# AllenNeuralDynamics/aind-exaspim-image-compression

Hardware: AMD Instinct MI355X
Metric: denoised+encoded voxels/s on 1024^3 uint16 (higher is better)
Workload: dtype f32

## Files before the change

aind-exaspim-image-compression_amd/csrc/bm_kernels.hip:

```cpp
#include "exabm4d_kernels.h"
#include <type_traits>

namespace exabm4d {

struct __attribute__((packed, aligned(4))) float4u {
    float x, y, z, w;
};

constexpr int TCZ = 8;
constexpr int NE = 6;
constexpr int NSTEP = SWIN * 2 * 4;
template <int TCY_, int TCX_>
struct TilePlan {
    static constexpr int TCY = TCY_, TCX = TCX_;
    static constexpr int TRY = TCY - 1, TRX = TCX - 1;
    static constexpr int PROWS = 4 * (TCY - 1) + 3 + NE;
    static_assert(TCY * TCX == 64, "one wave per cell layer");
};
template <int TCY_, int TCX_>
struct TileShape : TilePlan<TCY_, TCX_> {
    using Plan = TilePlan<TCY_, TCX_>;
    static constexpr int PCOLS = 4 * (TCX_ - 1) + 16;
    static constexpr int PSTR = TCX_ == 8 ? 56 : PCOLS;
    static constexpr int PCH = PSTR / 4;
    static constexpr int NDMA = (Plan::PROWS * PCH + 63) / 64;
    static constexpr int PLANE = (Plan::PROWS * PSTR + 3) / 4 * 4;
    static constexpr int PBUF = PLANE > 2144 ? PLANE : 2144;
    static_assert(PCOLS % 4 == 0 && PSTR % 4 == 0, "whole 16-byte chunks");
};

constexpr int CARRY_ROUND = (NE / 2) * SWIN * 64;
constexpr int CARRY_TILE = (NSTEP / 4) * 2 * CARRY_ROUND;
struct Carry {
    int on;
    int strip;
    uint32_t* buf;
    int* done;
    int* ticket;
    unsigned* status;
    int fault;
};
constexpr int CARRY_POLL_LIMIT = 1 << 23;
template <class T>
__device__ __forceinline__ void carry_prefetch(const T* src, T* dst, int lane) {
    static_assert(2 * CARRY_ROUND == 16 * 256 + 128, "two rounds = 16.5 KB");
#pragma unroll
    for (int i = 0; i < 16; i++)
        __builtin_amdgcn_global_load_lds((const __attribute__((address_space(1))) void*)(src + 256 * i + 4 * lane),
                                         (__attribute__((address_space(3))) void*)(dst + 256 * i), 16, 0, 17);
    if (lane < 32)
        __builtin_amdgcn_global_load_lds((const __attribute__((address_space(1))) void*)(src + 4096 + 4 * lane),
                                         (__attribute__((address_space(3))) void*)(dst + 4096), 16, 0, 17);
}
__device__ __forceinline__ void carry_wait_for(const int* done, int tiles, int lane, const Carry& carry) {
    if (lane == 0) {
        int polls = carry.fault ? CARRY_POLL_LIMIT : 0;
        while (__hip_atomic_load(done, __ATOMIC_RELAXED, __HIP_MEMORY_SCOPE_SYSTEM) < tiles) {
            if (++polls > CARRY_POLL_LIMIT) {
                __hip_atomic_fetch_or(carry.status, 1u, __ATOMIC_RELAXED, __HIP_MEMORY_SCOPE_SYSTEM);
                break;
            }
            __builtin_amdgcn_s_sleep(32);
        }
        if (carry.fault) __hip_atomic_fetch_or(carry.status, 1u, __ATOMIC_RELAXED, __HIP_MEMORY_SCOPE_SYSTEM);
    }
}
__device__ __forceinline__ int launch_position(const Carry& carry, int quota) {
    if (!carry.on) return (int)blockIdx.x;
    __shared__ int s_pos;
    if (threadIdx.x == 0) {
        const int xcc = (int)(__builtin_amdgcn_s_getreg((4 - 1) << 11 | 0 << 6 | 20) & 7);
        int pos = -1;
        for (int k = 0; k < 8 && pos < 0; k++) {
            const int c = (xcc + k) & 7;
            const int j = __hip_atomic_fetch_add(carry.ticket + c, 1, __ATOMIC_RELAXED, __HIP_MEMORY_SCOPE_AGENT);
            if (j < quota) pos = 8 * j + c;
        }
        s_pos = pos;
    }
    __syncthreads();
    return s_pos;
}

struct TileId {
    int tz, col, cols;
    int bi, ty, tx;
};
__device__ __forceinline__ bool tile_id(TileId& t, int tiles_y, int tiles_x, int xcd_q, int nbatch,
                                        const Carry& carry) {
    const int per = tiles_y * tiles_x;
    t.cols = per * nbatch;
    if (xcd_q) {
        const int lp = launch_position(carry, (int)(gridDim.x >> 3));
        const int s = lp < 0 ? -1 : xcd_slab_sync(lp, t.cols, xcd_q);
        if (s < 0) return false;
        t.tz = s / t.cols;
        t.col = s - t.tz * t.cols;
    } else {
        const int s = xcd_contiguous(blockIdx.x, gridDim.x);
        t.tz = s / per;
        t.col = (int)blockIdx.y * per + (s - t.tz * per);
    }
    t.bi = t.col / per;
    const int pos = t.col - t.bi * per;
    int ty, tx;
    if (carry.strip) {
        const int sidx = pos / (carry.strip * tiles_x), r = pos - sidx * (carry.strip * tiles_x);
        const int h = min(carry.strip, tiles_y - sidx * carry.strip);
        tx = r / h;
        ty = sidx * carry.strip + (r - tx * h);
    } else {
        ty = pos / tiles_x;
        tx = pos - ty * tiles_x;
    }
    t.ty = ty;
    t.tx = tx;
    return true;
}

__device__ __forceinline__ void list_admit(uint32_t (&list)[MAXG], uint32_t& thr, uint32_t keymax, uint32_t sbits,
                                           uint32_t code, bool valid) {
    uint32_t key = (sbits & KEY_DMASK) | code;
    key = valid ? key : KEY_EMPTY;
    if (__any(key < thr)) {
        const uint32_t kins = key < thr ? key : KEY_EMPTY;
        list_insert_inplace(list, kins);
        thr = min(list[MAXG - 1], keymax);
    }
}
__device__ __forceinline__ void list_store(uint32_t* out, uint32_t (&list)[MAXG]) {
    list[0] = list[0] == KEY_EMPTY ? 0u : list[0];
#pragma unroll
    for (int k = 0; k < MAXG; k += 4) {
        uint4 v = make_uint4(list[k], list[k + 1], list[k + 2], list[k + 3]);
        *reinterpret_cast<uint4*>(out + k) = v;
    }
}

template <class TS>
__global__ __launch_bounds__(512) void bm_tile_kernel(const float* __restrict__ vol_all, VolGeom g,
                                                      uint32_t keymax,
                                                      uint32_t* __restrict__ keys_all, int tiles_y,
                                                      int tiles_x, int guarded, int xcd_q, int nbatch, Carry carry) {
    constexpr int TCX = TS::TCX, TRX = TS::TRX, TRY = TS::TRY, PROWS = TS::PROWS,
                  PCOLS = TS::PCOLS, PSTR = TS::PSTR, PCH = TS::PCH, NDMA = TS::NDMA, PBUF = TS::PBUF;
    __shared__ __align__(16) float pbuf_all[TCZ][2][PBUF];
    __shared__ __align__(16) float lower0[2 * CARRY_ROUND + 64];

    TileId id;
    if (!tile_id(id, tiles_y, tiles_x, xcd_q, nbatch, carry)) return;
    const int tz = id.tz, col = id.col, cols = id.cols, bi = id.bi, ty = id.ty, tx = id.tx;
    const float* __restrict__ vol = vol_all + (size_t)bi * (size_t)g.nvox;
    uint32_t* __restrict__ keys = keys_all + (size_t)bi * (size_t)g.nref * MAXG;
    const int tid = threadIdx.x;
    const int lane = tid & 63;
    const int cx = lane % TCX, cy = lane / TCX, cz = __builtin_amdgcn_readfirstlane(tid >> 6);
    const int ix = TRX * tx + cx, iy = TRY * ty + cy;

    const size_t sy = (size_t)g.nx, sz = (size_t)g.nx * (size_t)g.ny;

    const int Ls = (carry.on ? TCZ : TCZ - 1) * tz;
    const float* carry_rd = reinterpret_cast<const float*>(carry.buf) + ((size_t)((tz + 1) & 1) * cols + col) * CARRY_TILE;
    float* carry_wr = reinterpret_cast<float*>(carry.buf) + ((size_t)(tz & 1) * cols + col) * CARRY_TILE;
    int* done_col = carry.done + col;

    const int qy = min(STEP * iy, g.ny - STEP), qx = min(STEP * ix, g.nx - STEP);
    const int Y0 = STEP * TRY * ty, X0 = STEP * TRX * tx - RAD;
    const bool xin = guarded || ((X0 >= 0) && (X0 + PCOLS - 1 <= g.nx - 1));

    const bool ref_yx = cx < TRX && cy < TRY && iy < g.ay && ix < g.ax;
    const int ry = STEP * iy, rx = STEP * ix;

    uint32_t xmask = 0;
#pragma unroll
    for (int d = 0; d < SWIN; d++)
        xmask |= ((rx + d - RAD >= 0) && (rx + d - RAD <= g.nx - BLK)) ? (1u << d) : 0u;

    const bool yin = (Y0 - RAD >= 0) && (Y0 + 1 + PROWS - 1 <= g.ny - 1);
    do {
    const int L = Ls + cz;
    const bool active = L <= g.az;
    const int iz = L - 1;
    const int qz = min(STEP * L, g.nz - STEP);
    const int Z0 = STEP * L;
    const bool lower_carried = carry.on && cz == 0 && tz > 0;
    const bool carries = carry.on && cz == TCZ - 1 && L + 1 <= g.az;
    const bool ref_ok = ref_yx && active && (cz > 0 || lower_carried);
    if ((lower_carried || carries) && tz > 0) carry_wait_for(done_col, tz, lane, carry);
    const int rz = STEP * iz;

    uint32_t list[MAXG];
#pragma unroll
    for (int k = 0; k < MAXG; k++) list[k] = KEY_EMPTY;
    uint32_t thr = keymax;

    auto step_plane = [&](int step, int& dylo) -> const float* {
        const int z = step & 3, pass = (step >> 2) & 1, dz = (step >> 3) - RAD;
        dylo = pass == 0 ? -RAD : 1;
        const int pz = min(max(Z0 + z + dz, 0), g.nz - 1);
        return vol + (size_t)pz * sz;
    };
    auto issue_dma = [&](int step, float* dst) {
        int dylo;
        const float* plane = step_plane(step, dylo);
        int l = lane;
        asm volatile("" : "+v"(l));
        if (yin) {
            const float* base = plane + (ptrdiff_t)(Y0 + dylo) * (ptrdiff_t)sy + X0;
#pragma unroll
            for (int i = 0; i < NDMA; i++) {
                const unsigned p = 64u * i + (unsigned)l;
                const unsigned r0 = (p * (65536u / PCH + 1u)) >> 16;
                const unsigned r = min(r0, (unsigned)(PROWS - 1));
                const unsigned q = min(p - r0 * PCH, (unsigned)(PCOLS / 4 - 1));
                const float* src = base + (r * (unsigned)sy + 4u * q);
                if (64 * i + 64 <= PROWS * PCH || p < (unsigned)(PROWS * PCH))
                    __builtin_amdgcn_global_load_lds(
                        (const __attribute__((address_space(1))) void*)src,
                        (__attribute__((address_space(3))) void*)(dst + 256 * i), 16, 0, 0);
            }
            return;
        }
#pragma unroll
        for (int i = 0; i < NDMA; i++) {
            const int p = 64 * i + l;
            const int r = min(p / PCH, PROWS - 1), q = min(p % PCH, PCOLS / 4 - 1);
            const int yy = min(max(Y0 + dylo + r, 0), g.ny - 1);
            const float* src = plane + (size_t)yy * sy + (X0 + 4 * q);
            if (64 * i + 64 <= PROWS * PCH || p < PROWS * PCH)
                __builtin_amdgcn_global_load_lds(
                    (const __attribute__((address_space(1))) void*)src,
                    (__attribute__((address_space(3))) void*)(dst + 256 * i), 16, 0, 0);
        }
    };
    auto stage_edge = [&](int step, float* dst) {
        int dylo;
        const float* plane = step_plane(step, dylo);
        for (int c = lane; c < PROWS * PCOLS; c += 64) {
            const int r = c / PCOLS, q = c - r * PCOLS;
            const int yy = min(max(Y0 + dylo + r, 0), g.ny - 1);
            const int xx = min(max(X0 + q, 0), g.nx - 1);
            dst[r * PSTR + q] = plane[(size_t)yy * sy + xx];
        }
    };

    if (!active) {
        for (int i = 0; i < (NSTEP / 4) * 4; i++) __syncthreads();
        break;
    }

    if (xin)
        issue_dma(0, pbuf_all[cz][0]);
    else
        stage_edge(0, pbuf_all[cz][0]);

    float acc[NE][SWIN];
#pragma unroll
    for (int e = 0; e < NE; e++)
#pragma unroll
        for (int d = 0; d < SWIN; d++) acc[e][d] = 0.0f;

#pragma unroll 1
    for (int step = 0; step < NSTEP; step++) {
        const int z = step & 3, pass = (step >> 2) & 1, dz = (step >> 3) - RAD;
        const int dylo = pass == 0 ? -RAD : 1;
        float* cur = pbuf_all[cz][step & 1];
        float* nxt = pbuf_all[cz][(step + 1) & 1];

        asm volatile("s_waitcnt vmcnt(0)" ::: "memory");
        float A[16];
#pragma unroll
        for (int y = 0; y < 4; y++) {
            const float4u t4 = *reinterpret_cast<const float4u*>(
                vol + (size_t)(qz + z) * sz + (size_t)(qy + y) * sy + qx);
            A[4 * y] = t4.x;
            A[4 * y + 1] = t4.y;
            A[4 * y + 2] = t4.z;
            A[4 * y + 3] = t4.w;
        }
        asm volatile("s_waitcnt vmcnt(0)" ::: "memory");
        if (xin && step + 1 < NSTEP) issue_dma(step + 1, nxt);
        if (lower_carried && z == 2) carry_prefetch(carry_rd + (size_t)(step >> 2) * 2 * CARRY_ROUND, lower0, lane);

        {
            const float* wrow = cur + (4 * cy) * PSTR + 4 * cx;
            float4 wq[4], wn[4];
#pragma unroll
            for (int j = 0; j < 4; j++) wq[j] = *reinterpret_cast<const float4*>(wrow + 4 * j);
#pragma unroll
            for (int rp = 0; rp < 3 + NE; rp++) {
                if (rp + 1 < 3 + NE) {
#pragma unroll
                    for (int j = 0; j < 4; j++)
                        wn[j] = *reinterpret_cast<const float4*>(wrow + (rp + 1) * PSTR + 4 * j);
                }
                asm volatile("" ::: "memory");
                const float w[16] = {wq[0].x, wq[0].y, wq[0].z, wq[0].w, wq[1].x, wq[1].y,
                                     wq[1].z, wq[1].w, wq[2].x, wq[2].y, wq[2].z, wq[2].w,
                                     wq[3].x, wq[3].y, wq[3].z, wq[3].w};
#pragma unroll
                for (int y = 0; y < 4; y++) {
                    const int e = rp - y;
                    if (e >= 0 && e < NE) {
#pragma unroll
                        for (int x = 0; x < 4; x++) {
                            const float a = A[4 * y + x];
#pragma unroll
                            for (int d = 0; d < SWIN; d++) {
                                const float t = a - w[d + x];
                                acc[e][d] = fmaf(t, t, acc[e][d]);
                            }
                        }
                    }
                }
#pragma unroll
                for (int j = 0; j < 4; j++) wq[j] = wn[j];
            }
        }
        asm volatile("" ::: "memory");

        if (z == 3) {
            const bool vz = (rz + dz >= 0) && (rz + dz <= g.nz - BLK);
            float* mine = cur + lane;
            const float* up_w = cur + lane;
            const float* lo_w = (cz > 0 ? pbuf_all[max(cz - 1, 0)][step & 1] : lower0) + lane;
            float* cslot = carry_wr + (size_t)((step >> 2) * 2) * CARRY_ROUND + lane;
#pragma unroll
            for (int e0 = 0; e0 < NE; e0 += NE / 2) {
#pragma unroll
                for (int e = e0; e < e0 + NE / 2; e++)
#pragma unroll
                    for (int d = 0; d < SWIN; d++) {
                        const float right = __int_as_float(__builtin_amdgcn_update_dpp(
                            0, __float_as_int(acc[e][d]), 0x101 , 0xF, 0xF, true));
                        mine[64 * ((e - e0) * SWIN + d)] = acc[e][d] + right;
                    }
                __syncthreads();
                if (ref_ok) {
#pragma unroll
                    for (int e = e0; e < e0 + NE / 2; e++) {
                        const int dy = dylo + e;
                        if (dy <= RAD) {
                            const bool vzy = vz && (ry + dy >= 0) && (ry + dy <= g.ny - BLK);
                            const uint32_t cbase =
                                1u + (uint32_t)(((dz + RAD) * SWIN + (dy + RAD)) * SWIN);
                            const bool self_row = (dz == 0) && (dy == 0);
#pragma unroll
                            for (int d = 0; d < SWIN; d++) {
                                const float* c0 = lo_w + (cz == 0 && e0 ? CARRY_ROUND : 0) + 64 * ((e - e0) * SWIN + d);
                                const float* c1 = up_w + 64 * ((e - e0) * SWIN + d);
                                float s0 = c0[0] + c0[TCX];
                                asm("" : "+v"(s0));
                                const float s1 = c1[0] + c1[TCX];
                                const float S = s0 + s1;
                                const uint32_t code = (d == RAD && self_row) ? 0u : cbase + d;
                                const bool valid = vzy && ((xmask >> d) & 1u);
                                list_admit(list, thr, keymax, __float_as_uint(S), code, valid);
                            }
                        }
                    }
                }
                __syncthreads();
                if (carries) {
#pragma unroll
                    for (int e = e0; e < e0 + NE / 2; e++)
#pragma unroll
                        for (int d = 0; d < SWIN; d++) {
                            const float right = __int_as_float(__builtin_amdgcn_update_dpp(
                                0, __float_as_int(acc[e][d]), 0x101 , 0xF, 0xF, true));
                            __hip_atomic_store(cslot + (e0 ? CARRY_ROUND : 0) + 64 * ((e - e0) * SWIN + d), acc[e][d] + right,
                                               __ATOMIC_RELAXED, __HIP_MEMORY_SCOPE_SYSTEM);
                        }
                }
            }
#pragma unroll
            for (int e = 0; e < NE; e++)
#pragma unroll
                for (int d = 0; d < SWIN; d++) acc[e][d] = 0.0f;
        }

        if (!xin && step + 1 < NSTEP) stage_edge(step + 1, nxt);
    }

    if (ref_ok) list_store(keys + ((size_t)((size_t)iz * g.gy + iy) * g.gx + ix) * MAXG, list);
    } while (false);

    if (carry.on) {
        asm volatile("s_waitcnt vmcnt(0)" ::: "memory");
        __syncthreads();
        if (threadIdx.x == 0) __hip_atomic_store(done_col, tz + 1, __ATOMIC_RELAXED, __HIP_MEMORY_SCOPE_SYSTEM);
    }
}

typedef short s16x2 __attribute__((ext_vector_type(2)));
template <int TCY_, int TCX_>
struct TileShape16 : TilePlan<TCY_, TCX_> {
    using Plan = TilePlan<TCY_, TCX_>;
    static constexpr int PCOLS = ((4 * TCX_ + 10 + 7) / 8) * 8;
    static constexpr int PSTR = TCX_ == 8 ? 56 : 80;
    static constexpr int PCH = PSTR / 8;
    static constexpr int NDMA = (Plan::PROWS * PCH + 63) / 64;
    static constexpr int PLANE_DW = NDMA * 256;
    static constexpr int XCH_DW = (NE / 2) * SWIN * 64;
    static constexpr int PBUF = PLANE_DW > XCH_DW ? PLANE_DW : XCH_DW;
    static_assert(PCOLS <= PSTR, "staged columns fit the row");
};

template <class TS>
__global__ __launch_bounds__(512) void bm_tile16_kernel(const uint16_t* __restrict__ vol_all, VolGeom g,
                                                        uint32_t keymax,
                                                        uint32_t* __restrict__ keys_all, int tiles_y,
                                                        int tiles_x, int xcd_q, int nbatch, Carry carry) {
    constexpr int TCX = TS::TCX, TRX = TS::TRX, TRY = TS::TRY, PROWS = TS::PROWS, PCOLS = TS::PCOLS,
                  PSTR = TS::PSTR, PCH = TS::PCH, NDMA = TS::NDMA, PBUF = TS::PBUF;
    __shared__ __align__(16) uint32_t pbuf_all[TCZ][2][PBUF];
    __shared__ __align__(16) uint32_t lower0[2 * CARRY_ROUND + 64];

    TileId id;
    if (!tile_id(id, tiles_y, tiles_x, xcd_q, nbatch, carry)) return;
    const int tz = id.tz, col = id.col, cols = id.cols, bi = id.bi, ty = id.ty, tx = id.tx;
    const uint16_t* __restrict__ vol = vol_all + (size_t)bi * (size_t)g.nvox;
    uint32_t* __restrict__ keys = keys_all + (size_t)bi * (size_t)g.nref * MAXG;
    const int tid = threadIdx.x;
    const int lane = tid & 63;
    const int cx = lane % TCX, cy = lane / TCX, cz = __builtin_amdgcn_readfirstlane(tid >> 6);
    const int ix = TRX * tx + cx, iy = TRY * ty + cy;
    const size_t sy = (size_t)g.nx, sz = (size_t)g.nx * (size_t)g.ny;

    const int Ls = (carry.on ? TCZ : TCZ - 1) * tz;
    const uint32_t* carry_rd = carry.buf + ((size_t)((tz + 1) & 1) * cols + col) * CARRY_TILE;
    uint32_t* carry_wr = carry.buf + ((size_t)(tz & 1) * cols + col) * CARRY_TILE;
    int* done_col = carry.done + col;

    const int qy = min(STEP * iy, g.ny - STEP), qx = min(STEP * ix, g.nx - STEP);
    const int Y0 = STEP * TRY * ty, X0 = STEP * TRX * tx - RAD - 1;
    const int ry = STEP * iy, rx = STEP * ix;
    const bool ref_yx = cx < TRX && cy < TRY && iy < g.ay && ix < g.ax;

    uint32_t xmask = 0;
#pragma unroll
    for (int d = 0; d < SWIN; d++)
        xmask |= ((rx + d - RAD >= 0) && (rx + d - RAD <= g.nx - BLK)) ? (1u << d) : 0u;
    const bool yin = (Y0 - RAD >= 0) && (Y0 + 1 + PROWS - 1 <= g.ny - 1);

    do {
    const int L = Ls + cz;
    const bool active = L <= g.az;
    const int iz = L - 1;
    const int qz = min(STEP * L, g.nz - STEP);
    const int Z0 = STEP * L;
    const bool lower_carried = carry.on && cz == 0 && tz > 0;
    const bool carries = carry.on && cz == TCZ - 1 && L + 1 <= g.az;
    const bool ref_ok = ref_yx && active && (cz > 0 || lower_carried);
    if ((lower_carried || carries) && tz > 0) carry_wait_for(done_col, tz, lane, carry);
    const int rz = STEP * iz;

    uint32_t list[MAXG];
#pragma unroll
    for (int k = 0; k < MAXG; k++) list[k] = KEY_EMPTY;
    uint32_t thr = keymax;

    auto issue_dma = [&](int step, uint32_t* dst) {
        const int z = step & 3, pass = (step >> 2) & 1, dz = (step >> 3) - RAD;
        const int dylo = pass == 0 ? -RAD : 1;
        const int pz = min(max(Z0 + z + dz, 0), g.nz - 1);
        const uint16_t* plane = vol + (size_t)pz * sz;
        int l = lane;
        asm volatile("" : "+v"(l));
#pragma unroll
        for (int i = 0; i < NDMA; i++) {
            const unsigned p = 64u * i + (unsigned)l;
            const unsigned r0 = (p * (65536u / PCH + 1u)) >> 16;
            const unsigned r = min(r0, (unsigned)(PROWS - 1));
            const unsigned q = min(p - r0 * PCH, (unsigned)(PCOLS / 8 - 1));
            const int yy = yin ? Y0 + dylo + (int)r : min(max(Y0 + dylo + (int)r, 0), g.ny - 1);
            const uint16_t* src = plane + (ptrdiff_t)yy * (ptrdiff_t)sy + (X0 + 8 * (int)q);
            __builtin_amdgcn_global_load_lds(
                (const __attribute__((address_space(1))) void*)src,
                (__attribute__((address_space(3))) void*)(dst + 256 * i), 16, 0, 0);
        }
    };

    if (!active) {
        for (int i = 0; i < (NSTEP / 4) * 4; i++) __syncthreads();
        break;
    }
    issue_dma(0, pbuf_all[cz][0]);

    int acc[NE][SWIN];
#pragma unroll
    for (int e = 0; e < NE; e++)
#pragma unroll
        for (int d = 0; d < SWIN; d++) acc[e][d] = 0;

    auto step_body = [&](auto NEc, const int step) {
        constexpr int NEP = decltype(NEc)::value;
        constexpr int NR0 = (NEP + 1) / 2;
        const int z = step & 3, dz = (step >> 3) - RAD;
        const int dylo = NEP == NE ? -RAD : 1;
        uint32_t* cur = pbuf_all[cz][step & 1];
        uint32_t* nxt = pbuf_all[cz][(step + 1) & 1];

        asm volatile("s_waitcnt vmcnt(0)" ::: "memory");
        uint2 A[4];
#pragma unroll
        for (int y = 0; y < 4; y++) {
            const uint32_t* ap = reinterpret_cast<const uint32_t*>(
                vol + (size_t)(qz + z) * sz + (size_t)(qy + y) * sy + qx);
            A[y] = make_uint2(ap[0], ap[1]);
        }
        asm volatile("s_waitcnt vmcnt(0)" ::: "memory");
        if (step + 1 < NSTEP) issue_dma(step + 1, nxt);
        if (lower_carried && z == 2) carry_prefetch(carry_rd + (size_t)(step >> 2) * 2 * CARRY_ROUND, lower0, lane);

        {
            const uint32_t* wrow = cur + ((4 * cy) * PSTR + 4 * cx) / 2;
            uint2 wq[4], wn[4];
#pragma unroll
            for (int j = 0; j < 4; j++) wq[j] = *reinterpret_cast<const uint2*>(wrow + 2 * j);
#pragma unroll
            for (int rp = 0; rp < 3 + NEP; rp++) {
                if (rp + 1 < 3 + NEP) {
#pragma unroll
                    for (int j = 0; j < 4; j++)
                        wn[j] = *reinterpret_cast<const uint2*>(wrow + (rp + 1) * (PSTR / 2) + 2 * j);
                }
                asm volatile("" ::: "memory");
                const uint32_t W[8] = {wq[0].x, wq[0].y, wq[1].x, wq[1].y, wq[2].x, wq[2].y, wq[3].x, wq[3].y};
                uint32_t Wo[7];
#pragma unroll
                for (int i = 0; i < 7; i++) Wo[i] = __builtin_amdgcn_alignbit(W[i + 1], W[i], 16);
#pragma unroll
                for (int y = 0; y < 4; y++) {
                    const int e = rp - y;
                    if (e >= 0 && e < NEP) {
#pragma unroll
                        for (int xp = 0; xp < 2; xp++) {
                            const s16x2 a = __builtin_bit_cast(s16x2, xp ? A[y].y : A[y].x);
#pragma unroll
                            for (int d = 0; d < SWIN; d++) {
                                const int j = 1 + 2 * xp + d;
                                const uint32_t wp = (j & 1) ? Wo[(j - 1) / 2] : W[j / 2];
                                const s16x2 t = __builtin_elementwise_sub_sat(a, __builtin_bit_cast(s16x2, wp));
                                acc[e][d] = __builtin_amdgcn_sdot2(t, t, acc[e][d], true);
                            }
                        }
                    }
                }
#pragma unroll
                for (int j = 0; j < 4; j++) wq[j] = wn[j];
            }
        }
        asm volatile("" ::: "memory");

        if (z == 3) {
            const bool vz = (rz + dz >= 0) && (rz + dz <= g.nz - BLK);
            uint32_t* mine = cur + lane;
            const uint32_t* up_w = cur + lane;
            const uint32_t* lo_w = (cz > 0 ? pbuf_all[max(cz - 1, 0)][step & 1] : lower0) + lane;
            uint32_t* cslot = carry_wr + (size_t)((step >> 2) * 2) * CARRY_ROUND + lane;
            auto pair_sum = [&](int e, int d) {
                const uint32_t c = min((uint32_t)acc[e][d], 1u << 27);
                const uint32_t right = (uint32_t)__builtin_amdgcn_update_dpp(
                    0, (int)c, 0x101 , 0xF, 0xF, true);
                return c + right;
            };
#pragma unroll
            for (int e0 = 0; e0 < NEP; e0 += NR0) {
#pragma unroll
                for (int e = e0; e < (e0 + NR0 < NEP ? e0 + NR0 : NEP); e++)
#pragma unroll
                    for (int d = 0; d < SWIN; d++) mine[64 * ((e - e0) * SWIN + d)] = pair_sum(e, d);
                __syncthreads();
                if (ref_ok) {
#pragma unroll
                    for (int e = e0; e < (e0 + NR0 < NEP ? e0 + NR0 : NEP); e++) {
                        uint32_t Sv[1][SWIN];
#pragma unroll
                        for (int d = 0; d < SWIN; d++) {
                            const uint32_t* c0 = lo_w + (cz == 0 && e0 ? CARRY_ROUND : 0) + 64 * ((e - e0) * SWIN + d);
                            const uint32_t* c1 = up_w + 64 * ((e - e0) * SWIN + d);
                            Sv[0][d] = (c0[0] + c0[TCX]) + (c1[0] + c1[TCX]);
                        }
                        asm volatile("" ::: "memory");
                        const int dy = dylo + e;
                        {
                            const bool vzy = vz && (ry + dy >= 0) && (ry + dy <= g.ny - BLK);
                            const uint32_t cbase =
                                1u + (uint32_t)(((dz + RAD) * SWIN + (dy + RAD)) * SWIN);
                            const bool self_row = (dz == 0) && (dy == 0);
#pragma unroll
                            for (int d = 0; d < SWIN; d++) {
                                const uint32_t S = Sv[0][d];
                                const uint32_t code = (d == RAD && self_row) ? 0u : cbase + d;
                                const bool valid = vzy && ((xmask >> d) & 1u);
                                list_admit(list, thr, keymax, __float_as_uint((float)S), code, valid);
                            }
                        }
                    }
                }
                __syncthreads();
                if (carries) {
                    uint32_t* cw = cslot + (size_t)(e0 ? CARRY_ROUND : 0);
#pragma unroll
                    for (int e = e0; e < (e0 + NR0 < NEP ? e0 + NR0 : NEP); e++)
#pragma unroll
                        for (int d = 0; d < SWIN; d++)
                            __hip_atomic_store(cw + 64 * ((e - e0) * SWIN + d), pair_sum(e, d), __ATOMIC_RELAXED,
                                               __HIP_MEMORY_SCOPE_SYSTEM);
                }
            }
#pragma unroll
            for (int e = 0; e < NE; e++)
#pragma unroll
                for (int d = 0; d < SWIN; d++) acc[e][d] = 0;
        }
    };
#pragma unroll 1
    for (int step = 0; step < NSTEP; step++) {
        if (((step >> 2) & 1) == 0)
            step_body(std::integral_constant<int, NE>{}, step);
        else
            step_body(std::integral_constant<int, NE - 1>{}, step);
    }

    if (ref_ok) list_store(keys + ((size_t)((size_t)iz * g.gy + iy) * g.gx + ix) * MAXG, list);
    } while (false);

    if (carry.on) {
        asm volatile("s_waitcnt vmcnt(0)" ::: "memory");
        __syncthreads();
        if (threadIdx.x == 0) __hip_atomic_store(done_col, tz + 1, __ATOMIC_RELAXED, __HIP_MEMORY_SCOPE_SYSTEM);
    }
}

__global__ __launch_bounds__(64) void bm_generic_kernel(const float* __restrict__ vol_all,
                                                        VolGeom g, uint32_t keymax,
                                                        uint32_t* __restrict__ keys_all,
                                                        int only_unaligned) {
    __shared__ float rb[BVOX];
    const float* __restrict__ vol = vol_all + (size_t)blockIdx.y * (size_t)g.nvox;
    uint32_t* __restrict__ keys = keys_all + (size_t)blockIdx.y * (size_t)g.nref * MAXG;

    const long long r = blockIdx.x;
    const int ix = (int)(r % g.gx), iy = (int)((r / g.gx) % g.gy),
              iz = (int)(r / ((long long)g.gx * g.gy));
    if (only_unaligned && iz < g.az && iy < g.ay && ix < g.ax) return;
    const int rz = grid_pos(iz, g.az, g.nz), ry = grid_pos(iy, g.ay, g.ny),
              rx = grid_pos(ix, g.ax, g.nx);
    const size_t sy = (size_t)g.nx, sz = (size_t)g.nx * (size_t)g.ny;
    const int lane = threadIdx.x;

    for (int i = lane; i < BVOX; i += 64) {
        const int bx = i & 7, by = (i >> 3) & 7, bz = i >> 6;
        rb[i] = vol[(size_t)(rz + bz) * sz + (size_t)(ry + by) * sy + (rx + bx)];
    }
    __syncthreads();

    uint32_t list[MAXG];
#pragma unroll
    for (int k = 0; k < MAXG; k++) list[k] = KEY_EMPTY;

    for (int c = lane; c < NCAND; c += 64) {
        const int dx = c % SWIN - RAD, dy = (c / SWIN) % SWIN - RAD, dz = c / (SWIN * SWIN) - RAD;
        const int pz = rz + dz, py = ry + dy, px = rx + dx;
        const bool valid = pz >= 0 && pz <= g.nz - BLK && py >= 0 && py <= g.ny - BLK && px >= 0 &&
                           px <= g.nx - BLK;
        uint32_t key = KEY_EMPTY;
        if (valid) {
            const float* __restrict__ b = vol + (size_t)pz * sz + (size_t)py * sy + px;
            float cell[8];
#pragma unroll 1
            for (int kc = 0; kc < 8; kc++) {
                const int kz = kc >> 2, ky = (kc >> 1) & 1, kx = kc & 1;
                float acc = 0.0f;
#pragma unroll 1
                for (int z = 0; z < 4; z++)
#pragma unroll
                    for (int y = 0; y < 4; y++) {
                        const int bz = 4 * kz + z, by = 4 * ky + y;
                        const float* bp = b + (size_t)bz * sz + (size_t)by * sy + 4 * kx;
                        const float* ap = rb + (bz * 8 + by) * 8 + 4 * kx;
#pragma unroll
                        for (int x = 0; x < 4; x++) {
                            const float t = ap[x] - bp[x];
                            acc = fmaf(t, t, acc);
                        }
                    }
                cell[kc] = acc;
            }
            const float lo = (cell[0] + cell[1]) + (cell[2] + cell[3]);
            const float hi = (cell[4] + cell[5]) + (cell[6] + cell[7]);
            const float S = lo + hi;
            key = (__float_as_uint(S) & KEY_DMASK) | disp_code(dz, dy, dx);
            if (key >= keymax) key = KEY_EMPTY;
        }
        list_insert(list, key);
    }

    uint32_t* out = keys + (size_t)r * MAXG;
    for (int k = 0; k < MAXG; k++) {
        uint32_t m = list[0];
#pragma unroll
        for (int off = 32; off >= 1; off >>= 1) m = min(m, (uint32_t)__shfl_xor((int)m, off));
        if (list[0] == m && m != KEY_EMPTY) {
#pragma unroll
            for (int i = 0; i < MAXG - 1; i++) list[i] = list[i + 1];
            list[MAXG - 1] = KEY_EMPTY;
        }
        if (lane == 0) out[k] = (k == 0 && m == KEY_EMPTY) ? 0u : m;
    }
}


using Cube = TilePlan<8, 8>;
using Flat = TilePlan<4, 16>;
static bool flat_tiles(const VolGeom& g) {
    auto tiles = [&](int try_, int trx) {
        return (long long)((g.ay + try_ - 1) / try_) * ((g.ax + trx - 1) / trx);
    };
    return tiles(Flat::TRY, Flat::TRX) < tiles(Cube::TRY, Cube::TRX);
}
BmPlan bm_plan(const VolGeom& g, int batch, const BmOpts& opt) {
    BmPlan p = {};
    if (g.az <= 0 || g.ay <= 0 || g.ax <= 0) return p;
    p.flat = flat_tiles(g) ? 1 : 0;
    const int try_ = p.flat ? Flat::TRY : Cube::TRY, trx = p.flat ? Flat::TRX : Cube::TRX;
    p.ty = (g.ay + try_ - 1) / try_;
    p.tx = (g.ax + trx - 1) / trx;
    const long long cols = (long long)p.ty * p.tx * batch;
    const int tz7 = (g.az + TCZ - 2) / (TCZ - 1), tz8 = g.az / TCZ + 1;
    const bool slab = opt.xcd_mode != 0 && cols >= 512;
    const bool worth = tz8 >= 2 && tz8 < tz7 && slab;
    const size_t need = 2 * (size_t)cols * CARRY_TILE * sizeof(uint32_t) + ((size_t)cols + 64) * sizeof(int);
    p.carry = (opt.carry != 0 && (worth || (opt.carry == 2 && tz8 >= 2)) && need <= ((size_t)16 << 30)) ? 1 : 0;
    p.carry_bytes = p.carry ? need : 0;
    p.tz = p.carry ? tz8 : tz7;
    p.xq = (p.carry || (slab && p.tz >= 2)) ? (int)((cols + 7) / 8) : 0;
    p.strip = (opt.xcd_mode >= 2 && p.xq) ? opt.xcd_mode : 0;
    p.fault = opt.carry_fault;
    return p;
}

hipError_t launch_blockmatch(const float* vol, const VolGeom& g, int batch, uint32_t keymax,
                             uint32_t* keys, hipStream_t stream, int force_generic, int guarded,
                             const uint16_t* vol16, const BmPlan& p, void* carry_mem, unsigned* status) {
    if (p.carry && (!carry_mem || !status)) return hipErrorInvalidValue;
    if (!force_generic && g.az > 0 && g.ay > 0 && g.ax > 0) {
        Carry carry;
        carry.strip = p.strip;
        carry.on = p.carry;
        carry.buf = static_cast<uint32_t*>(carry_mem);
        const size_t cols = (size_t)p.ty * p.tx * (size_t)batch;
        carry.done = p.carry ? reinterpret_cast<int*>(carry.buf + 2 * cols * CARRY_TILE) : nullptr;
        carry.ticket = p.carry ? carry.done + cols : nullptr;
        carry.status = status;
        carry.fault = p.fault;
        if (p.carry) {
            hipError_t e = hipMemsetAsync(carry.done, 0, (cols + 8) * sizeof(int), stream);
            if (e != hipSuccess) return e;
        }
        const dim3 grid((unsigned)(p.xq ? 8 * p.xq * p.tz : p.tz * p.ty * p.tx), (unsigned)(p.xq ? 1 : batch));
        auto launch = [&](auto plan) {
            using Shape16 = TileShape16<decltype(plan)::TCY, decltype(plan)::TCX>;
            using Shape = TileShape<decltype(plan)::TCY, decltype(plan)::TCX>;
            if (vol16)
                hipLaunchKernelGGL(bm_tile16_kernel<Shape16>, grid, dim3(512), 0, stream, vol16, g, keymax, keys,
                                   p.ty, p.tx, p.xq, batch, carry);
            else
                hipLaunchKernelGGL(bm_tile_kernel<Shape>, grid, dim3(512), 0, stream, vol, g, keymax, keys, p.ty,
                                   p.tx, guarded, p.xq, batch, carry);
        };
        if (p.flat)
            launch(Flat{});
        else
            launch(Cube{});
        hipError_t e = hipGetLastError();
        if (e != hipSuccess) return e;
    }
    const bool unaligned = g.gz != g.az || g.gy != g.ay || g.gx != g.ax;
    if (force_generic || unaligned) {
        dim3 grid((unsigned)g.nref, (unsigned)batch);
        hipLaunchKernelGGL(bm_generic_kernel, grid, dim3(64), 0, stream, vol, g, keymax, keys,
                           force_generic ? 0 : 1);
        return hipGetLastError();
    }
    return hipSuccess;
}

}
```

Measured before the change: 1.924 billion.

## Prefetch next cell plane and hand-schedule LDS row reads in bm_tile16

Moves the per-step global load of the reference cell plane one step ahead, so it is issued alongside the next DMA and no longer stalls on a separate vmcnt(0) wait each step. Replaces the compiler-generated LDS row loads with inline ds_read2_b64 and explicit lgkmcnt waits, so the next row is fetched while the current one is processed. Also adds optional s_memtime stamp instrumentation behind a macro. The hand-written waits tie correctness to exact instruction ordering, and holding the prefetched plane in registers adds register pressure.

```diff
diff --git a/aind-exaspim-image-compression_amd/csrc/bm_kernels.hip b/aind-exaspim-image-compression_amd/csrc/bm_kernels.hip
--- a/aind-exaspim-image-compression_amd/csrc/bm_kernels.hip
+++ b/aind-exaspim-image-compression_amd/csrc/bm_kernels.hip
@@ -1,11 +1,39 @@
 #include "exabm4d_kernels.h"
 #include <type_traits>
+#include <utility>
+
+#ifndef EXABM4D_BM_HANDWAIT
+#define EXABM4D_BM_HANDWAIT 1
+#endif
 
 namespace exabm4d {
+
+#ifdef EXABM4D_BM_STAMPS
+__device__ unsigned long long g_bm_stamps[8];
+__device__ __forceinline__ unsigned long long bm_stamp() {
+    unsigned long long t;
+    __builtin_amdgcn_sched_barrier(0);
+    asm volatile("s_memtime %0\n\ts_waitcnt lgkmcnt(0)" : "=s"(t)::"memory");
+    __builtin_amdgcn_sched_barrier(0);
+    return t;
+}
+#define BM_STAMP(var) const unsigned long long var = bm_stamp()
+#define BM_STAMP_ADD(i, a, b) st[i] += (b) - (a)
+#else
+#define BM_STAMP(var)
+#define BM_STAMP_ADD(i, a, b)
+#endif
 
 struct __attribute__((packed, aligned(4))) float4u {
     float x, y, z, w;
 };
+template <class F, int... I>
+__device__ __forceinline__ void static_for(F&& f, std::integer_sequence<int, I...>) {
+    (f(std::integral_constant<int, I>{}), ...);
+}
+__device__ __forceinline__ uint32_t lds_byte_address(const void* p) {
+    return (uint32_t)(uintptr_t)(__attribute__((address_space(3))) const void*)p;
+}
 
 constexpr int TCZ = 8;
 constexpr int NE = 6;
@@ -393,6 +421,9 @@
 }
 
 typedef short s16x2 __attribute__((ext_vector_type(2)));
+typedef uint32_t u32x2 __attribute__((ext_vector_type(2)));
+typedef uint32_t u32x4 __attribute__((ext_vector_type(4)));
+typedef u32x4 u32x4a8 __attribute__((aligned(8)));
 template <int TCY_, int TCX_>
 struct TileShape16 : TilePlan<TCY_, TCX_> {
     using Plan = TilePlan<TCY_, TCX_>;
@@ -426,6 +457,10 @@
     const int cx = lane % TCX, cy = lane / TCX, cz = __builtin_amdgcn_readfirstlane(tid >> 6);
     const int ix = TRX * tx + cx, iy = TRY * ty + cy;
     const size_t sy = (size_t)g.nx, sz = (size_t)g.nx * (size_t)g.ny;
+#ifdef EXABM4D_BM_STAMPS
+    unsigned long long st[8] = {};
+    const unsigned long long tk0 = bm_stamp();
+#endif
 
     const int Ls = (carry.on ? TCZ : TCZ - 1) * tz;
     const uint32_t* carry_rd = carry.buf + ((size_t)((tz + 1) & 1) * cols + col) * CARRY_TILE;
@@ -452,13 +487,28 @@
     const bool lower_carried = carry.on && cz == 0 && tz > 0;
     const bool carries = carry.on && cz == TCZ - 1 && L + 1 <= g.az;
     const bool ref_ok = ref_yx && active && (cz > 0 || lower_carried);
-    if ((lower_carried || carries) && tz > 0) carry_wait_for(done_col, tz, lane, carry);
+    {
+        BM_STAMP(c0);
+        if ((lower_carried || carries) && tz > 0) carry_wait_for(done_col, tz, lane, carry);
+        BM_STAMP(c1);
+        BM_STAMP_ADD(6, c0, c1);
+    }
     const int rz = STEP * iz;
 
     uint32_t list[MAXG];
 #pragma unroll
     for (int k = 0; k < MAXG; k++) list[k] = KEY_EMPTY;
     uint32_t thr = keymax;
+
+    u32x2 An[4];
+    auto load_cell_plane = [&](int step) {
+#pragma unroll
+        for (int y = 0; y < 4; y++) {
+            const uint32_t* ap = reinterpret_cast<const uint32_t*>(
+                vol + (size_t)(qz + (step & 3)) * sz + (size_t)(qy + y) * sy + qx);
+            An[y] = u32x2{ap[0], ap[1]};
+        }
+    };
 
     auto issue_dma = [&](int step, uint32_t* dst) {
         const int z = step & 3, pass = (step >> 2) & 1, dz = (step >> 3) - RAD;
@@ -486,6 +536,10 @@
         break;
     }
     issue_dma(0, pbuf_all[cz][0]);
+    if (EXABM4D_BM_HANDWAIT) {
+        load_cell_plane(0);
+        asm volatile("" ::"v"(An[0]), "v"(An[1]), "v"(An[2]), "v"(An[3]));
+    }
 
     int acc[NE][SWIN];
 #pragma unroll
@@ -501,32 +555,59 @@
         uint32_t* cur = pbuf_all[cz][step & 1];
         uint32_t* nxt = pbuf_all[cz][(step + 1) & 1];
 
+        BM_STAMP(t0);
         asm volatile("s_waitcnt vmcnt(0)" ::: "memory");
-        uint2 A[4];
-#pragma unroll
-        for (int y = 0; y < 4; y++) {
-            const uint32_t* ap = reinterpret_cast<const uint32_t*>(
-                vol + (size_t)(qz + z) * sz + (size_t)(qy + y) * sy + qx);
-            A[y] = make_uint2(ap[0], ap[1]);
-        }
-        asm volatile("s_waitcnt vmcnt(0)" ::: "memory");
+        BM_STAMP(t1);
+        if (!EXABM4D_BM_HANDWAIT) {
+            load_cell_plane(step);
+            asm volatile("s_waitcnt vmcnt(0)" ::: "memory");
+        }
+        const u32x2 A[4] = {An[0], An[1], An[2], An[3]};
+#ifdef EXABM4D_BM_STAMPS
+        if (!EXABM4D_BM_HANDWAIT) asm volatile("" ::"v"(A[0]), "v"(A[1]), "v"(A[2]), "v"(A[3]));
+#endif
+        BM_STAMP(t2);
         if (step + 1 < NSTEP) issue_dma(step + 1, nxt);
         if (lower_carried && z == 2) carry_prefetch(carry_rd + (size_t)(step >> 2) * 2 * CARRY_ROUND, lower0, lane);
+        if (EXABM4D_BM_HANDWAIT) {
+            if (step + 1 < NSTEP) load_cell_plane(step + 1);
+            asm volatile("" ::: "memory");
+        }
+        BM_STAMP(t3);
 
         {
             const uint32_t* wrow = cur + ((4 * cy) * PSTR + 4 * cx) / 2;
-            uint2 wq[4], wn[4];
-#pragma unroll
-            for (int j = 0; j < 4; j++) wq[j] = *reinterpret_cast<const uint2*>(wrow + 2 * j);
-#pragma unroll
-            for (int rp = 0; rp < 3 + NEP; rp++) {
-                if (rp + 1 < 3 + NEP) {
-#pragma unroll
-                    for (int j = 0; j < 4; j++)
-                        wn[j] = *reinterpret_cast<const uint2*>(wrow + (rp + 1) * (PSTR / 2) + 2 * j);
+            const uint32_t wrow_lds = lds_byte_address(wrow);
+            auto read_row = [&](auto rc, u32x4& lo, u32x4& hi) {
+                constexpr int r = decltype(rc)::value;
+                constexpr int O = r * (PSTR / 4);
+                static_assert(O + 3 < 256, "ds_read2_b64 offsets are 8 bits");
+                if (EXABM4D_BM_HANDWAIT) {
+                    asm volatile("ds_read2_b64 %0, %2 offset0:%3 offset1:%4\n\t"
+                                 "ds_read2_b64 %1, %2 offset0:%5 offset1:%6"
+                                 : "=&v"(lo), "=&v"(hi)
+                                 : "v"(wrow_lds), "n"(O), "n"(O + 1), "n"(O + 2), "n"(O + 3));
+                } else {
+                    lo = *reinterpret_cast<const u32x4a8*>(wrow + r * (PSTR / 2));
+                    hi = *reinterpret_cast<const u32x4a8*>(wrow + r * (PSTR / 2) + 4);
                 }
+            };
+            auto await_row = [&](u32x4& lo, u32x4& hi) {
+                if (EXABM4D_BM_HANDWAIT) asm volatile("s_waitcnt lgkmcnt(0)" : "+v"(lo), "+v"(hi));
+            };
+            u32x4 q0, q1;
+            read_row(std::integral_constant<int, 0>{}, q0, q1);
+            await_row(q0, q1);
+#ifdef EXABM4D_BM_STAMPS
+            if (!EXABM4D_BM_HANDWAIT) asm volatile("" : "+v"(q0), "+v"(q1));
+#endif
+            BM_STAMP(t4);
+            static_for([&](auto rc) {
+                constexpr int rp = decltype(rc)::value;
+                u32x4 n0, n1;
+                if constexpr (rp + 1 < 3 + NEP) read_row(std::integral_constant<int, rp + 1>{}, n0, n1);
                 asm volatile("" ::: "memory");
-                const uint32_t W[8] = {wq[0].x, wq[0].y, wq[1].x, wq[1].y, wq[2].x, wq[2].y, wq[3].x, wq[3].y};
+                const uint32_t W[8] = {q0.x, q0.y, q0.z, q0.w, q1.x, q1.y, q1.z, q1.w};
                 uint32_t Wo[7];
 #pragma unroll
                 for (int i = 0; i < 7; i++) Wo[i] = __builtin_amdgcn_alignbit(W[i + 1], W[i], 16);
@@ -547,11 +628,19 @@
                         }
                     }
                 }
-#pragma unroll
-                for (int j = 0; j < 4; j++) wq[j] = wn[j];
-            }
-        }
-        asm volatile("" ::: "memory");
+                if constexpr (rp + 1 < 3 + NEP) {
+                    await_row(n0, n1);
+                    q0 = n0;
+                    q1 = n1;
+                }
+            }, std::make_integer_sequence<int, 3 + NEP>{});
+            asm volatile("" ::: "memory");
+            BM_STAMP(t5);
+            BM_STAMP_ADD(0, t0, t1);
+            BM_STAMP_ADD(1, t1, t2);
+            BM_STAMP_ADD(2, t3, t4);
+            BM_STAMP_ADD(3, t4, t5);
+        }
 
         if (z == 3) {
             const bool vz = (rz + dz >= 0) && (rz + dz <= g.nz - BLK);
@@ -571,7 +660,9 @@
                 for (int e = e0; e < (e0 + NR0 < NEP ? e0 + NR0 : NEP); e++)
 #pragma unroll
                     for (int d = 0; d < SWIN; d++) mine[64 * ((e - e0) * SWIN + d)] = pair_sum(e, d);
+                BM_STAMP(b0);
                 __syncthreads();
+                BM_STAMP(b1);
                 if (ref_ok) {
 #pragma unroll
                     for (int e = e0; e < (e0 + NR0 < NEP ? e0 + NR0 : NEP); e++) {
@@ -599,7 +690,12 @@
                         }
                     }
                 }
+                BM_STAMP(b2);
                 __syncthreads();
+                BM_STAMP(b3);
+                BM_STAMP_ADD(4, b0, b1);
+                BM_STAMP_ADD(5, b1, b2);
+                BM_STAMP_ADD(4, b2, b3);
                 if (carries) {
                     uint32_t* cw = cslot + (size_t)(e0 ? CARRY_ROUND : 0);
 #pragma unroll
@@ -628,11 +724,28 @@
     } while (false);
 
     if (carry.on) {
+        BM_STAMP(c0);
         asm volatile("s_waitcnt vmcnt(0)" ::: "memory");
         __syncthreads();
+        BM_STAMP(c1);
+        BM_STAMP_ADD(6, c0, c1);
         if (threadIdx.x == 0) __hip_atomic_store(done_col, tz + 1, __ATOMIC_RELAXED, __HIP_MEMORY_SCOPE_SYSTEM);
     }
-}
+#ifdef EXABM4D_BM_STAMPS
+    st[7] = bm_stamp() - tk0;
+    if (lane == 0)
+        for (int i = 0; i < 8; i++) atomicAdd(&g_bm_stamps[i], st[i]);
+#endif
+}
+
+#ifdef EXABM4D_BM_STAMPS
+extern "C" void exabm4d_debug_bm_stamps(unsigned long long* out, int reset) {
+    unsigned long long z[8] = {};
+    (void)hipDeviceSynchronize();
+    (void)hipMemcpyFromSymbol(out, HIP_SYMBOL(g_bm_stamps), sizeof(z));
+    if (reset) (void)hipMemcpyToSymbol(HIP_SYMBOL(g_bm_stamps), z, sizeof(z));
+}
+#endif
 
 __global__ __launch_bounds__(64) void bm_generic_kernel(const float* __restrict__ vol_all,
                                                         VolGeom g, uint32_t keymax,
```

Result: faster. 1.944 billion (median of 6 runs) (+1.0%).
